# nlamprian/ICP

Hardware: AMD Instinct MI355X
Metric: ICP iterations/sec at |F|=|M|=16384, |R|=256 (higher is better)
Workload: dtype f32

## Files before the change

icp_amd/csrc/icp_search.h:

```cpp
#pragma once
#include "icp_kernels.h"

static __device__ __forceinline__ float sum4 (float4 v) { return ((v.x + v.y) + v.z) + v.w; }
static __device__ __forceinline__ uint32_t ks_hole_bit (float4 mg) { return (mg.x == 0.f && mg.y == 0.f && mg.z == 0.f) ? 0x80000000u : 0u; }

#define KS_SPLIT LPQ
#define KS_QPW (64 / KS_SPLIT)
#define KS_TILE 1024u
#ifndef ICP_S2_DEPTH16
#define ICP_S2_DEPTH16 8u
#endif
#ifndef ICP_S2_UNCOND
#define ICP_S2_UNCOND 128u
#endif
#ifndef ICP_S1_ORIGIN_LIST
#define ICP_S1_ORIGIN_LIST 1
#endif
#ifndef ICP_OL_STAGED_MIN
#define ICP_OL_STAGED_MIN 32u
#endif
#ifndef ICP_S1_SEED
#define ICP_S1_SEED 1
#endif
#ifndef ICP_S1_REJECT_MIN_NR
#define ICP_S1_REJECT_MIN_NR 1024u
#endif

typedef float float2v __attribute__ ((ext_vector_type (2)));

struct k_search_args {
    const float *gM, *gR; icp_reg_state *gst; const double *gmom;
    uint32_t m, nr, side, tpr_magic, nb, check_flags;
    icp_params p;
};
#define KS_PARAMS_OFFSET offsetof (k_search_args, p)
static_assert (KS_PARAMS_OFFSET == 4 * 8 + 6 * 4, "k_search: four pointers and six dwords in front of icp_params");
static_assert (KS_PARAMS_OFFSET % alignof (icp_params) == 0, "kernel-argument layout: icp_params follows the scalars without padding");
static __device__ __forceinline__ const icp_params *ks_params_from_kernarg ()
{
    unsigned long long a_ = (unsigned long long) __builtin_amdgcn_kernarg_segment_ptr () + KS_PARAMS_OFFSET;
    asm volatile ("" : "+s"(a_));
    return (const icp_params *) (const icp_params __attribute__ ((address_space (4))) *) a_;
}
#ifndef ICP_HOME_MODE
#define ICP_HOME_MODE 1
#endif

// ... 210 lines not shown
static __device__ __forceinline__ void fused_moment_task (uint32_t nb, uint32_t ps, uint32_t &k, uint32_t &g, bool &live)
{
    constexpr uint32_t nrow = NT / 16;
    const uint32_t row = threadIdx.x >> 4, ng = (nb + 127u) / 128u, ntask = ICP_NMOM * ng;
    const uint32_t task = min (ps * nrow + row, ntask - 1u);
    if (ng == 1) { k = task; g = 0u; } else if (ng == 2) { k = task >> 1; g = task & 1u; } else { k = task / ng; g = task - k * ng; }
    live = ps * nrow + row < ntask;
}
template <int NT>
static __device__ __forceinline__ void fused_moment_loads (const double *mom, uint32_t nb, uint32_t ps, double *a)
{
    uint32_t k, g; bool live;
    fused_moment_task<NT> (nb, ps, k, g, live);
    const double *src = mom + (size_t) k * nb;
    const uint32_t l = threadIdx.x & 15u;
#pragma unroll
    for (int q = 0; q < 8; ++q) a[q] = 0.0;
    if (live) {
        if (nb & 127u) {
#pragma unroll
            for (int q = 0; q < 8; ++q) {
                const uint32_t i = g * 128u + l + 16u * q;
                const double t = src[min (i, nb - 1u)];
                a[q] = (i < nb) ? t : 0.0;
            }
        } else {
#pragma unroll
            for (int q = 0; q < 8; ++q) a[q] = src[g * 128u + l + 16u * q];
        }
    }
}

struct ff_no_hook { __device__ void operator() (const float *) const {} };
template <int NG, int NT, int ROT, bool LEAN = false, bool REJ = false, typename AFTER = ff_no_hook>
static __device__ bool fused_finalize_block (const icp_params &p, const double *mom, uint32_t nb, uint32_t check, uint32_t sv,
                                             const double *a0, icp_fin_result *res, double (*s_l1)[NG], double *s_t,
                                             const double *gl1 = nullptr, icp_reg_state *direct = nullptr, AFTER after = AFTER (),
                                             uint32_t pending_unless_done = 1u, unsigned long long *mirror = nullptr, bool progress = false,
                                             icp_reg_state *final_dst = nullptr, icp_reg_state *host_dst = nullptr, icp_reg_state *prev_dst = nullptr)
{
    constexpr uint32_t nrow = NT / 16;
    const uint32_t tid = threadIdx.x, lane = tid & 63u, l = tid & 15u, row = tid >> 4;
    const uint32_t ng = (nb + 127u) / 128u;
    const uint32_t ntask = ICP_NMOM * ng, npass = (ntask + nrow - 1u) / nrow;
    auto pass = [&] (uint32_t ps, const double *a) {
        uint32_t k, g; bool live;
        fused_moment_task<NT> (nb, ps, k, g, live);
        FF_STAMP (13)
        double v = row_tree8_d (a);
        if (nb == 1) v = a[0];
        if (ng == 2) {
            const double o = __shfl_down (v, 16);
            if (l == 0 && !(row & 1u) && live) s_t[k] = (v + 0.0) + (o + 0.0);
        } else if (l == 0 && live) { if (ng == 1) s_t[k] = v; else s_l1[k][g] = v; }
    };
    if (gl1 == nullptr) {
        pass (0u, a0);
        for (uint32_t ps = 1; ps < npass; ++ps) {
            double a[8];
            fused_moment_loads<NT> (mom, nb, ps, a);
            pass (ps, a);
        }
    }
    if (check && __builtin_amdgcn_readlane ((int) sv, (int) ICP_ST_DW (done))) return false;
    FF_STAMP (9)
    if (ng > 2) {
        __syncthreads ();
        if (row < 20) {
            const uint32_t k = min (row, (uint32_t) ICP_NMOM - 1u);
            double a[8];
#pragma unroll
            for (int q = 0; q < 8; ++q) {
// ... 75 lines not shown
                        *reinterpret_cast<f4u *> (dst + 4) = f4u { Tprev[4], Tprev[5], Tprev[6], Tprev[7] };
                    }
                    if (mirror) {
                        if (done) {
                            if (final_dst) store_image (final_dst);
                            if (host_dst) { store_image (host_dst); __threadfence_system (); }
                            icp_mirror_store (mirror, ICP_MIRROR_WORD (p.epoch, kprev + 1u, 1u) | (host_dst ? ICP_MIRROR_FINAL : 0ull));
                            if (progress && p.run_flag) {
                                p.run_flag[blockIdx.y] = p.epoch;
                                if (p.track_seq) __hip_atomic_store (p.track_seq, p.seq_value, __ATOMIC_RELEASE, __HIP_MEMORY_SCOPE_AGENT);
                            }
                        } else if (progress) icp_mirror_store (mirror, ICP_MIRROR_WORD (p.epoch, kprev + 1u, 0u));
                    }
                }
            }
        } else if (lane == 0) {
            float Tn[8], Rn[9];
            if (none) icp_identity_step (Tprev, Rprev, S, means, Tk, Tn, Rn, Rk, iters);
            else icp_compose_pure (Tprev, Rprev, Tk, Rkin, ROT != 1, Tn, Rn, Rk);
#pragma unroll
            for (int k = 0; k < 8; ++k) { res->T[k] = Tn[k]; res->Tk[k] = Tk[k]; res->means[k] = means[k]; }
#pragma unroll
            for (int k = 0; k < 9; ++k) { res->R[k] = Rn[k]; res->Rk[k] = Rk[k]; }
#pragma unroll
            for (int k = 0; k < 11; ++k) res->S[k] = S[k];
            res->sum_w = sw; res->pm_iters = (uint32_t) iters; res->k = kprev + 1u; res->pad0 = 0.f; res->pending = 0u;
            res->reserved0 = 0u; res->reserved1 = 0u;
            res->done = (p.check && icp_check_converged (Tk, p.tan_half_thr, p.trans_thr)) ? 1u : 0u;
            if (prev_dst) {
#pragma unroll
                for (int k = 0; k < 8; ++k) prev_dst->T[k] = Tprev[k];
            }
        }
    }
    __syncthreads ();
    return true;
}

static __device__ __forceinline__ void fin_result_to_state (const icp_fin_result *res, icp_reg_state *st, uint32_t pending)
{
    static_assert (sizeof (icp_reg_state) / 4 <= 64, "the state is published by one wave");
    const uint32_t t = threadIdx.x;
    if (t < sizeof (icp_reg_state) / 4) {
        uint32_t v = reinterpret_cast<const uint32_t *> (res)[t];
        if (t == offsetof (icp_reg_state, pending) / 4) v = pending;
        reinterpret_cast<uint32_t *> (st)[t] = v;
    }
}

template <int LPQ>
static __device__ __forceinline__ void ks_list_tail (const char *XQb, uint32_t o, uint32_t je, uint32_t alast, uint32_t cb0, uint32_t ntrips, float qx, float qy, float qz,
                                                     float qr, float qg, float qb, float alpha, float dr, uint32_t b, uint32_t lane, uint32_t ss, float &best2, uint32_t &bj)
{
    const float2v vq_xr = { qx, qr }, vq_yg = { qy, qg }, vq_zb = { qz, qb };
    constexpr uint32_t CPT = 16u / KS_SPLIT, BD = KS_SPLIT == 16 ? 2u : 1u;
    const uint32_t nch = (je - o + 15u) >> 4, nchw = (ntrips + CPT - 1u) / CPT;
    const icp_params *pl = ks_params_from_kernarg ();
    typedef float4 __attribute__ ((address_space (1))) *gf4;
    const float4 *LBq = (const float4 *) (gf4) pl->LB + (size_t) b * 3u * pl->nlb + 3u * (o >> 4);
    const float inf_ = __builtin_inff ();
    float lim = (alpha > 0.f && dr >= 0.f && dr < inf_) ? __uint_as_float (__float_as_uint (dr) + 1u) : inf_;
    const bool bounds = alpha > 0.f;
    for (uint32_t cb = cb0; cb < nchw; cb += BD * KS_SPLIT) {
        lim = fminf (lim, ks_grp_min_f<KS_SPLIT> (best2));
        float4 bx[BD][3];
#pragma unroll
        for (uint32_t j = 0; j < BD; ++j) {
// ... 124 lines not shown
        const bool odd = (lane & 2u) != 0u;
        const unsigned long long keep = odd ? k4[2 * j + 1] : k4[2 * j], send = odd ? k4[2 * j] : k4[2 * j + 1];
        k2[j] = min64 (keep, xchg_dpp (send, std::integral_constant<int, 0x4E> {}));
    }
    {
        const bool odd = (lane & 4u) != 0u;
        const unsigned long long keep = odd ? k2[1] : k2[0], send = odd ? k2[0] : k2[1];
        k1 = min64 (keep, xchg_lane (send, lane ^ 4u));
    }
    k1 = min64 (k1, xchg_lane (k1, lane ^ 8u));
    k1 = min64 (k1, xchg_lane (k1, lane ^ 16u));
    k1 = min64 (k1, xchg_lane (k1, lane ^ 32u));
    k1 = xchg_lane (k1, (lane & 56u) | (lane >> 3));
    dmin = __uint_as_float ((uint32_t) (k1 >> 32)); jmin = (uint32_t) k1;
    {
        uint32_t nl = (je - o + 7u) >> 3;
        nl = max (nl, (uint32_t) __builtin_amdgcn_update_dpp (0, (int) nl, 0x140, 0xF, 0xF, true));
        nl = max (nl, (uint32_t) __builtin_amdgcn_update_dpp ((int) nl, (int) nl, 0x142, 0xA, 0xF, false));
        nl = max (nl, (uint32_t) __builtin_amdgcn_update_dpp ((int) nl, (int) nl, 0x143, 0xC, 0xF, false));
        const uint32_t ntrips = (uint32_t) __builtin_amdgcn_readlane ((int) nl, 63);
        if (__builtin_expect (ntrips > ICP_S2W_UNCOND / 8u, 0)) {
            const uint32_t ss = lane & 7u;
            float best2 = dmin; uint32_t bj = 0xFFFFFFFFu;
            const float4 a4 = s_qa[qe], c4 = s_qc[qe];
            ks_list_tail<8> (XQb, o, je, (max (je, 1u) - 1u) << 5, ICP_S2W_UNCOND / 16u, ntrips, a4.x, a4.y, a4.z, c4.x, c4.y, c4.z, alpha, dr, b, lane, ss, best2, bj);
            const uint32_t pos = bj != 0xFFFFFFFFu ? min (o + ss + bj * 8u, max (je, 1u) - 1u) : jmin;
            const float d2 = ks_grp_min_f<8> (best2);
            jmin = ks_grp_min_u<8> (best2 == d2 ? pos : 0xFFFFFFFFu);
            dmin = d2;
        }
    }
}

template <int LPQ>
static __device__ __forceinline__ void ks_stage2_lanes (const char *XQb, uint32_t o, uint32_t n, bool valid, float qx, float qy, float qz, float qr, float qg, float qb,
                                                        float alpha, float dr, uint32_t b, uint32_t lane, uint32_t ss, float &dmin, uint32_t &jmin)
{
    float best2 = __builtin_inff (); uint32_t bj = 0xFFFFFFFFu;
    const float2v vq_xr = { qx, qr }, vq_yg = { qy, qg }, vq_zb = { qz, qb };
    {
        constexpr uint32_t KS_DEPTH = (KS_SPLIT == 16) ? ICP_S2_DEPTH16 : 4u;
        const uint32_t je = valid ? o + n : o;
        uint32_t nl = (je - o + KS_SPLIT - 1u) / KS_SPLIT;
        if (KS_SPLIT == 8) nl = max (nl, (uint32_t) __builtin_amdgcn_update_dpp (0, (int) nl, 0x140, 0xF, 0xF, true));
        nl = max (nl, (uint32_t) __builtin_amdgcn_update_dpp ((int) nl, (int) nl, 0x142, 0xA, 0xF, false));
        nl = max (nl, (uint32_t) __builtin_amdgcn_update_dpp ((int) nl, (int) nl, 0x143, 0xC, 0xF, false));
        const uint32_t ntrips = (uint32_t) __builtin_amdgcn_readlane ((int) nl, 63);
        const uint32_t alast = (max (je, 1u) - 1u) << 5;
        constexpr uint32_t KS_UNC = ICP_S2_UNCOND / KS_SPLIT;
        const uint32_t ntr0 = (ICP_S2_UNCOND == 0u || ntrips <= 2u * KS_UNC) ? ntrips : KS_UNC;
        for (uint32_t tb = 0; tb < ntr0; tb += KS_DEPTH) {
            const uint32_t a0 = (o + ss + tb * KS_SPLIT) << 5, nt = min (KS_DEPTH, ntr0 - tb);
            float4 g[KS_DEPTH], c[KS_DEPTH];
#pragma unroll
            for (uint32_t t = 0; t < KS_DEPTH; ++t) {
                if (t >= nt) break;
                const char *rec = XQb + min (a0 + t * (KS_SPLIT * 32u), alast);
                g[t] = *reinterpret_cast<const float4 *> (rec); c[t] = *reinterpret_cast<const float4 *> (rec + 16);
            }
#pragma unroll
            for (uint32_t t = 0; t < KS_DEPTH; ++t) {
                if (t >= nt) break;
                KS_CAND (g[t], c[t], tb + t);
            }
        }
        if (__builtin_expect (ntrips > ntr0, 0))
            ks_list_tail<LPQ> (XQb, o, je, alast, ICP_S2_UNCOND / 16u, ntrips, qx, qy, qz, qr, qg, qb, alpha, dr, b, lane, ss, best2, bj);
        if (bj != 0xFFFFFFFFu) bj = min (o + ss + bj * KS_SPLIT, max (je, 1u) - 1u);
        if (je == o) { best2 = __builtin_inff (); bj = 0xFFFFFFFFu; }
    }
    dmin = ks_grp_min_f<KS_SPLIT> (best2);
    jmin = ks_grp_min_u<KS_SPLIT> (best2 == dmin ? bj : 0xFFFFFFFFu);
}

template <bool FUSED, bool CHAIN, int MINW, int LPQ, bool OWNER, bool PRUNE, bool REJ>
static __device__ __forceinline__ void ks_epilogue (const icp_params &p, float4 *s_qa, uint4 *s_qb, const float4 *s_qc, const uint32_t *s_slot, double (*s_mom)[64], float *s_w, const float4 *R4, const char *XQb,
                                                    uint32_t b, uint32_t m, uint32_t nr, uint32_t check_flags, uint32_t tid, uint32_t lane, uint32_t slice, uint32_t tile_id,
                                                    uint32_t qe, uint32_t ss, uint32_t i, bool valid, uint32_t o, uint32_t n, uint32_t rstar, float dr, float dmin, uint32_t jmin,
                                                    float qx, float qy, float qz)
{
    if (ss == 0u) {
        const bool empty = (n == 0u);
        s_qa[qe] = make_float4 (qx, qy, qz, empty ? dr : dmin);
        s_qb[qe] = make_uint4 (empty ? rstar : ((jmin == 0xFFFFFFFFu) ? o : jmin), rstar, (valid ? 1u : 0u) | (empty ? 2u : 0u), i);
    }
    __syncthreads ();
    if (slice == 0u) {
        const float4 qa = s_qa[lane]; const uint4 qb = s_qb[lane];
        const uint32_t eo = (PRUNE && ICP_S1_ORIGIN_LIST) ? s_slot[lane] : lane;
        const bool v = (qb.z & 1u) != 0u, empty = (qb.z & 2u) != 0u;
        const float ex = qa.x, ey = qa.y, ez = qa.z, d = p.dist_scale * qa.w;
        const uint32_t ei = qb.w;
        float w = 0.f, f0 = 0.f, f1 = 0.f, f2 = 0.f;
        bool acc = v;
        if (v) {
            uint32_t id;
            if (empty) {
                const float4 nn = R4[2 * (size_t) qb.x];
                const uint32_t *rsrc = p.rep_src;
                if constexpr (MINW == 4) {
                    typedef uint32_t __attribute__ ((address_space (1))) *gu32;
                    rsrc = (const uint32_t *) (gu32) ks_params_from_kernarg ()->rep_src;
                }
                id = rsrc[(size_t) b * nr + qb.x]; f0 = nn.x; f1 = nn.y; f2 = nn.z;
            } else {
                const char *rec = XQb + (qb.x << 5);
                const float4 wg = *reinterpret_cast<const float4 *> (rec), wc = *reinterpret_cast<const float4 *> (rec + 16);
                f0 = wg.x; f1 = wg.z; f2 = wc.x; id = __float_as_uint (wc.z);
            }
            w = p.weighted ? 100.f / (100.f + d) : 1.f;
            if constexpr (REJ) {
                bool rej = false;
                if (p.reject & 1u)
                    rej = (__float_as_uint (s_qc[lane].w) >> 31) != 0u || (f0 == 0.f && f1 == 0.f && f2 == 0.f);
                if (p.reject & ICP_REJECT_DIST_ON) {
                    const float gx = ex - f0, gy = ey - f1, gz = ez - f2;
                    rej = rej || !(((gx * gx + gy * gy) + gz * gz) <= p.reject_d2);
                }
                if (rej) { w = 0.f; acc = false; }
            }
            icp_dist_id di; di.dist = d; di.id = id;
            const icp_params *pe = &p;
            if constexpr (MINW == 2 && !OWNER) {
                            pe = ks_params_from_kernarg ();
            }
            typedef char __attribute__ ((address_space (1))) *gchar;
            char *o_nn = (char *) (gchar) reinterpret_cast<char *> (pe->nn_id + (size_t) b * m), *o_pf = (char *) (gchar) reinterpret_cast<char *> (pe->PF + (size_t) b * m);
            char *o_pm = (char *) (gchar) reinterpret_cast<char *> (pe->PM + (size_t) b * m), *o_rid = (char *) (gchar) reinterpret_cast<char *> (pe->rid + (size_t) b * m);
            const bool emit = !FUSED || (check_flags & 8u);
            if (emit) {
                *reinterpret_cast<icp_dist_id *> (o_nn + (ei << 3)) = di;
                *reinterpret_cast<float4 *> (o_pf + (ei << 4)) = make_float4 (f0, f1, f2, w);
                *reinterpret_cast<float4 *> (o_pm + (ei << 4)) = make_float4 (ex, ey, ez, d);
            }
            if (emit || PRUNE) *reinterpret_cast<uint32_t *> (o_rid + (ei << 2)) = qb.y;
        }
        if constexpr (FUSED) {
            double W = (double) w;
            double g0 = acc ? (double) f0 : 0.0, g1 = acc ? (double) f1 : 0.0, g2 = acc ? (double) f2 : 0.0;
            double q0 = (double) ex, q1 = (double) ey, q2 = (double) ez;
            if (!acc) { W = 0.0; q0 = q1 = q2 = 0.0; }
// ... 82 lines not shown
                                                     uint32_t gt_lg1, uint32_t ss, uint32_t t0_, uint32_t npair_, uint32_t cmask_, float &best, uint32_t &bid)
{
    const uint32_t ngt_ = (npair_ + KS_SPLIT - 1u) / KS_SPLIT;
    const float2v vqx = { qx, qx }, vqy = { qy, qy }, vqz = { qz, qz }, vqr = { qr, qr }, vqg = { qg, qg }, vqb = { qb, qb };
    const float2v va = { alpha, alpha };
    for (uint32_t t = 0; t * KS_SPLIT < ngt_; ++t) {
        unsigned long long bal = __ballot ((cmask_ >> t) & 1u);
        if (bal == 0ull) continue;
        bal |= bal >> 32; bal |= bal >> 16;
        if (KS_SPLIT == 8) bal |= bal >> 8;
        uint32_t need = (uint32_t) bal & ((1u << KS_SPLIT) - 1u);
        while (need) {
            const uint32_t sg = (uint32_t) __builtin_ctz (need);
            need &= need - 1u;
            const uint32_t gl = sg + KS_SPLIT * t;
            const uint32_t P = (KS_SPLIT == 8 && gt_lg1) ? (((4u * (gl >> (gt_lg1 - 1u)) + (ss >> 1)) << gt_lg1) + 2u * (gl & ((1u << (gt_lg1 - 1u)) - 1u)) + (ss & 1u))
                                                          : gl * KS_SPLIT + ss;
            if (P < npair_) {
                const uint32_t P3 = pair0 + __umul24 (P, 3u);
                float4 A = s_pair[P3], B = s_pair[P3 + 1], C = s_pair[P3 + 2];
                float2v x = { A.x, A.y }, y = { A.z, A.w }, z = { B.x, B.y }, r = { B.z, B.w }, g = { C.x, C.y }, bb = { C.z, C.w };
                float2v dx = vqx - x, dy = vqy - y, dz = vqz - z, dr = vqr - r, dg = vqg - g, db = vqb - bb;
                float2v geo = __builtin_elementwise_fma (dz, dz, __builtin_elementwise_fma (dy, dy, dx * dx));
                float2v pho = __builtin_elementwise_fma (db, db, __builtin_elementwise_fma (dg, dg, dr * dr));
                float2v d = __builtin_elementwise_fma (va, pho, geo);
                const uint32_t r0 = t0_ + 2u * P;
                if (d.x < best) { best = d.x; bid = r0; }
                if (d.y < best) { best = d.y; bid = r0 + 1u; }
            }
        }
    }
}

template <bool FUSED, bool CHAIN, int MINW, int LPQ, bool OWNER = false, int ROT = 1, int TILE = 1024, bool SINGLE = false, bool S2W = false, bool HOSTRUN = false,
          bool REJ = false>
__global__ __launch_bounds__ (64 * LPQ, TILE == 256 ? 8 : MINW) void k_search (const float *gM, const float *gR, icp_reg_state *gst, const double *gmom,
                                                              uint32_t m, uint32_t nr, uint32_t side, uint32_t tpr_magic,
                                                              uint32_t nb, uint32_t check_flags, icp_params p)
{
    constexpr uint32_t KT = (uint32_t) TILE;
    constexpr bool MASKED = (TILE == 256) && !SINGLE && (MINW == 4);
    if constexpr (SINGLE) __builtin_assume (nr <= KT);
    if constexpr (MASKED) __builtin_assume (nr > KT && nr <= 32u * KT);
    const uint32_t b = blockIdx.y, check = check_flags & 1u;
    icp_reg_state *st = (CHAIN && !(check_flags & 2u)) ? gst + (size_t) b * 2 : gst + b;
#ifdef ICP_DBG_STAMPS
    { const uint32_t tid = threadIdx.x; unsigned long long t_; asm volatile ("s_memtime %0\n\ts_waitcnt lgkmcnt(0)" : "=s"(t_) :: "memory");
      KS_STAMP_STORE (8) }
#endif

    constexpr uint32_t NBUF = MASKED ? 2u : 1u, PB = 3u * KT / 2u, BB = 2u * (KT / 16u);
    __shared__ float4 s_pair[NBUF * PB];
    __shared__ uint2 s_on[(MASKED && OWNER) ? 1 : KT];
    __shared__ uint32_t s_tmask;
    __shared__ uint32_t s_ovote;
    __shared__ float4 s_box[NBUF * BB];
    __shared__ float4 s_tbox[(MINW == 4 && !SINGLE) ? 2 * 32 : 2];
    __shared__ float s_w[64];
    __shared__ float4 s_qc[64];
    __shared__ float4 s_qa[64];
    __shared__ uint4 s_qb[64];
    __shared__ uint32_t s_slot[(ICP_S1_SEED && ICP_S1_ORIGIN_LIST && MINW == 4) ? 64 : 1];
    __shared__ double s_mom[FUSED ? ICP_NMOM : 1][64];
    __shared__ icp_fin_result s_fin;
    __shared__ double s_l1[CHAIN ? ICP_NMOM : 1][CHAIN ? 32 : 1];
    __shared__ double s_t[ICP_NMOM];

    const uint32_t tid = threadIdx.x, lane = tid & 63u;
    const uint32_t slice = __builtin_amdgcn_readfirstlane (tid >> 6);
    const uint32_t qe = slice * KS_QPW + lane / KS_SPLIT, ss = lane & (KS_SPLIT - 1u);
    const bool qwave = CHAIN ? slice == 0u : slice == KS_SPLIT - 1u;
    constexpr bool OWNER_LISTS = OWNER && MINW == 2;
    const uint32_t tile_id = OWNER_LISTS ? blockIdx.x : (FUSED && (MINW == 2 || (check_flags & 64u))) ? ks_tile_of_block (blockIdx.x, nb) : blockIdx.x;
    const uint32_t iq = OWNER_LISTS ? blockIdx.x * 64u + lane :
                        FUSED ? fused_query_index (m, side, tpr_magic, tile_id, lane)
                              : (blockIdx.x >> 1) * 128u + 2u * lane + (blockIdx.x & 1u);

    const float4 *M4 = reinterpret_cast<const float4 *> (gM + (size_t) b * m * 8);
    const float4 *R4 = reinterpret_cast<const float4 *> (gR + (size_t) b * nr * 8);

    uint32_t sv = OWNER ? 0u : state_load_lanes (st);
    uint32_t run_over = 0u;
    if constexpr (CHAIN) {
        static_assert (ICP_ST_DW (T) == 0 && ICP_ST_DW (Tk) == 8 && ICP_ST_DW (R) == 16 && ICP_ST_DW (Rk) == 25 && ICP_ST_DW (reserved0) == 60, "state layout");
        if (check_flags & 16u) {
            constexpr unsigned long long ones = (1ull << 3) | (1ull << 7) | (1ull << 11) | (1ull << 15) | (1ull << 16) | (1ull << 20) | (1ull << 24) |
                                                (1ull << 25) | (1ull << 29) | (1ull << 33);
            if (lane < ICP_ST_DW (reserved0)) sv = ((ones >> lane) & 1ull) ? 0x3F800000u : 0u;
        }
    }
    double ma0[8];
    if constexpr (CHAIN) fused_moment_loads<64 * LPQ> (gmom + (size_t) b * 2 * ICP_NMOM * nb, nb, 0u, ma0);
    float *s_pairf = reinterpret_cast<float *> (s_pair);
    const uint32_t tn0 = min (KT, nr);
    float4 rg[2], rc[2]; uint2 ron[2];
    uint32_t ht = 0u, tnH = 0u;
#pragma unroll
    for (int u = 0; u < 2; ++u) {
        uint32_t k = tid + (uint32_t) u * 64u * KS_SPLIT;
// ... 42 lines not shown
    }
    const float4 *GBt = p.GB + (size_t) b * 2 * (p.n16 + p.n1k) + (KS_SPLIT == 8 ? 0u : 2u * p.n16);
    const uint32_t nbox0 = 2u * ((tn0 + 2u * KS_SPLIT - 1u) / (2u * KS_SPLIT));
    float4 boxv = make_float4 (0.f, 0.f, 0.f, 0.f);
    if (!MASKED && prune && tid < nbox0) boxv = GBt[tid];
    const uint32_t nboxH = 2u * ((tnH + 2u * KS_SPLIT - 1u) / (2u * KS_SPLIT));
    if (MASKED && ICP_HOME_MODE != 3 && prune && tid < nboxH) boxv = GBt[2u * (ht * KT / (2u * KS_SPLIT)) + tid];
    float T[8];
#pragma unroll
    for (int k = 0; k < 8; ++k) T[k] = state_lane_f (sv, ICP_ST_DW (T) + k);
    if constexpr (PRUNE && !OWNER) {
        if (seed_cell != 0xFFFFFFFFu && __builtin_amdgcn_readlane ((int) sv, (int) ICP_ST_DW (k)) == 0) seed = seed_cell | (ICP_S1_ORIGIN_LIST ? 0x40000000u : 0u);
    }
    icp_reg_state *sout = CHAIN ? p.cst + (size_t) b * 2 + (p.slot ^ 1u) : st;
    if constexpr (!OWNER && !CHAIN) {
        const uint32_t done_ = (uint32_t) __builtin_amdgcn_readlane ((int) sv, (int) ICP_ST_DW (done));
        if (p.hmirror && blockIdx.x == 0 && tid == 0 && !(FUSED && done_))
            icp_mirror_store (p.hmirror + b, ICP_MIRROR_WORD (p.epoch, (uint32_t) __builtin_amdgcn_readlane ((int) sv, (int) ICP_ST_DW (k)), done_));
    }
    if constexpr (CHAIN && HOSTRUN) { if (run_over) return; }
    if (!OWNER && check && __builtin_amdgcn_readlane ((int) sv, (int) ICP_ST_DW (done))) {
        if constexpr (CHAIN) {
            if (blockIdx.x == 0 && tid < sizeof (icp_reg_state) / 4) reinterpret_cast<uint32_t *> (sout)[tid] = sv;
        }
        return;
    }
    if constexpr (!S2W) asm volatile ("" : "+v"(mgv), "+v"(mcv));
    float4 mg = make_float4 (mgv.x, mgv.y, mgv.z, mgv.w), mc = make_float4 (mcv.x, mcv.y, mcv.z, mcv.w);
    if (iq >= m) { mg = make_float4 (0.f, 0.f, 0.f, 1.f); mc = mg; }
    uint32_t hbit = 0u;
    if constexpr (REJ && !OWNER) { hbit = ks_hole_bit (mg); if constexpr (CHAIN) asm volatile ("" : "+v"(hbit)); }
    const float4 *XQ4 = reinterpret_cast<const float4 *> (p.XQ + (size_t) b * m * 8);
    const char *XQb = reinterpret_cast<const char *> (XQ4);
#pragma unroll
    for (int u = 0; u < 2; ++u) {
        uint32_t k = tid + (uint32_t) u * 64u * KS_SPLIT;
        if (!MASKED && k < tn0) {
            float *dst = s_pairf + (k >> 1) * 12u + (k & 1u);
            dst[0] = rg[u].x; dst[2] = rg[u].y; dst[4] = rg[u].z; dst[6] = rc[u].x; dst[8] = rc[u].y; dst[10] = rc[u].z;
            if constexpr (!OWNER && !MASKED) s_on[k] = ron[u];
        }
    }
    if (!MASKED && prune && tid < nbox0) s_box[tid] = boxv;
    auto home_to_lds = [&] () {
        if (tid < tnH) {
            float *dst = s_pairf + PB * 4u + (tid >> 1) * 12u + (tid & 1u);
            dst[0] = rg[0].x; dst[2] = rg[0].y; dst[4] = rg[0].z; dst[6] = rc[0].x; dst[8] = rc[0].y; dst[10] = rc[0].z;
        }
        if (prune && tid < nboxH) s_box[BB + tid] = boxv;
    };
    if constexpr (MASKED) {
        if (ICP_HOME_MODE == 1) home_to_lds ();
        if constexpr (!OWNER) { if (tid < tnH) s_on[tid] = ron[0]; }
    }
    if (MASKED && tid == 0) s_tmask = 0u;
    if (PRUNE && ICP_S1_ORIGIN_LIST && tid == 0) s_ovote = 0u;
    if constexpr (MINW == 4 && !SINGLE) {
        if (prune && nr > KT && tid < 2u * p.n1k) s_tbox[tid] = p.GB[(size_t) b * 2 * (p.n16 + p.n1k) + 2u * p.n16 + tid];
    }
    bool handed = false;
    if constexpr (CHAIN) {
        const bool pending = __builtin_amdgcn_readlane ((int) sv, (int) ICP_ST_DW (pending)) != 0;
        if (pending) {
            auto hand_over = [&] (const float *Tn) {
                float tx, ty, tz;
                icp_transform_point (Tn, mg.x, mg.y, mg.z, tx, ty, tz);
                s_qa[lane] = make_float4 (tx, ty, tz, __uint_as_float (iq));
                s_qc[lane] = make_float4 (mc.x, mc.y, mc.z, __uint_as_float (seed | hbit));
            };
            fused_finalize_block<32, 64 * LPQ, ROT, true, REJ> (p, gmom + (size_t) b * 2 * ICP_NMOM * nb, nb, 0u, sv, ma0, &s_fin, s_l1, s_t, nullptr,
                                                           blockIdx.x == 0 ? sout : nullptr, hand_over, 1u,
                                                           (HOSTRUN && blockIdx.x == 0 && p.hmirror) ? p.hmirror + b : nullptr, HOSTRUN, HOSTRUN ? p.st + b : nullptr,
                                                           (HOSTRUN && p.hstate) ? p.hstate + b : nullptr, (HOSTRUN && p.st_prev) ? p.st_prev + b : nullptr);
            handed = true;
            KS_STAMP (9)
            if (s_fin.done) return;
        } else if (blockIdx.x == 0 && tid < sizeof (icp_reg_state) / 4) {
            reinterpret_cast<uint32_t *> (sout)[tid] = (tid == offsetof (icp_reg_state, pending) / 4) ? 1u : sv;
        }
    }
    if (qwave && !handed) {
        float tx = mg.x, ty = mg.y, tz = mg.z;
        if constexpr (!OWNER) icp_transform_point (T, mg.x, mg.y, mg.z, tx, ty, tz);
        if constexpr (PRUNE && ICP_S1_ORIGIN_LIST) {
            const bool hole = mg.x == 0.f && mg.y == 0.f && mg.z == 0.f;
            const float4 ha = make_float4 (tx, ty, tz, __uint_as_float (iq)), hc = make_float4 (mc.x, mc.y, mc.z, __uint_as_float (hole ? (seed | 0x80000000u) : seed));
            s_qa[lane] = ha; s_qc[lane] = hc; s_slot[lane] = lane;
            const unsigned long long hb = __ballot (hole);
            if (__builtin_expect (hb != 0ull, 0)) {
                const unsigned long long lt = (1ull << lane) - 1ull;
                const uint32_t pos = hole ? 64u - (uint32_t) __builtin_popcountll (hb) + (uint32_t) __builtin_popcountll (hb & lt) : (uint32_t) __builtin_popcountll (~hb & lt);
                s_qa[pos] = ha; s_qc[pos] = hc; s_slot[pos] = lane;
            }
        } else {
            s_qa[lane] = make_float4 (tx, ty, tz, __uint_as_float (iq));
            s_qc[lane] = make_float4 (mc.x, mc.y, mc.z, __uint_as_float (seed | hbit));
        }
    }
    float qx = 0.f, qy = 0.f, qz = 0.f, qr = 0.f, qg = 0.f, qb = 0.f;
    uint32_t i = 0u; bool valid = false;
    const float alpha = p.a;
    KS_STAMP (0)

    float best = __builtin_inff (), s1_lim = __builtin_inff (); uint32_t bid = 0xFFFFFFFFu;
    uint32_t n_origin = 0u;
    if constexpr (MASKED) {
// ... 162 lines not shown
                float4 A = s_pair[3 * P], B = s_pair[3 * P + 1], C = s_pair[3 * P + 2];
                float2v x = { A.x, A.y }, y = { A.z, A.w }, z = { B.x, B.y }, r = { B.z, B.w }, g = { C.x, C.y }, bb = { C.z, C.w };
                float2v dx = vqx - x, dy = vqy - y, dz = vqz - z, dr = vqr - r, dg = vqg - g, db = vqb - bb;
                float2v geo = __builtin_elementwise_fma (dz, dz, __builtin_elementwise_fma (dy, dy, dx * dx));
                float2v pho = __builtin_elementwise_fma (db, db, __builtin_elementwise_fma (dg, dg, dr * dr));
                float2v d = __builtin_elementwise_fma (va, pho, geo);
                const uint32_t r0 = t0 + 2u * P;
                if (d.x < best) { best = d.x; bid = r0; }
                if (d.y < best) { best = d.y; bid = r0 + 1u; }
            }
        }
    }
    KS_STAMP (14)
    if constexpr (PRUNE && ICP_S1_ORIGIN_LIST) {
        if (prune && __builtin_expect (n_origin != 0u, 0))
            ks_origin_section<KS_SPLIT, PB> (s_pair, &s_ovote, n_origin, nr, b, slice, tid, qx, qy, qz, qr, qg, qb, alpha, s1_lim, lane, ss, best, bid);
    }
    KS_KEEP (best, bid)
    KS_STAMP (2)
    const float dr = ks_grp_min_f<KS_SPLIT> (best);
    const bool named = PRUNE ? (best == dr && dr < __builtin_inff ()) : (best == dr);
    uint32_t rstar = ks_grp_min_u<KS_SPLIT> (named ? bid : 0xFFFFFFFFu);
    if (rstar == 0xFFFFFFFFu) rstar = 0u;
    if constexpr (OWNER_LISTS) {
        ks_owner_lists_tail (p, s_qb, b, m, nb, lane, slice, qe, ss, valid, rstar);
        return;
    } else if constexpr (OWNER) {
        if (ss == 0u && valid) p.owner[(size_t) b * m + i] = rstar;
        return;
    }
    KS_KEEP (dr, rstar)
    KS_STAMP (3)
    uint32_t o, n;
    if constexpr (MINW == 2) { const uint2 on = s_on[rstar]; o = on.x; n = on.y; }
    else if constexpr (MASKED) {
        if (rstar / KT == ht) { const uint2 on = s_on[rstar - ht * KT]; o = on.x; n = on.y; asm volatile ("" : "+v"(o), "+v"(n)); }
        else { o = gO[rstar]; n = gN[rstar]; }
    }
    else if (nr <= KT) { const uint2 on = s_on[rstar]; o = on.x; n = on.y; asm volatile ("" : "+v"(o), "+v"(n)); }
    else { o = gO[rstar]; n = gN[rstar]; }

    float dmin; uint32_t jmin;
    if constexpr (S2W) {
        static_assert (MINW == 4 && LPQ == 8 && !OWNER, "lanes = candidates: the dense search variants");
        ks_stage2_wave (XQb, o, n, valid, rstar, qx, qy, qz, qr, qg, qb, alpha, dr, b, lane, s_qa, s_qc, qe, dmin, jmin);
    } else ks_stage2_lanes<LPQ> (XQb, o, n, valid, qx, qy, qz, qr, qg, qb, alpha, dr, b, lane, ss, dmin, jmin);
    KS_KEEP (dmin, jmin)
    KS_STAMP (5)
    ks_epilogue<FUSED, CHAIN, MINW, LPQ, OWNER, PRUNE, REJ> (p, s_qa, s_qb, s_qc, s_slot, s_mom, s_w, R4, XQb, b, m, nr, check_flags, tid, lane, slice, tile_id, qe, ss, i, valid, o, n, rstar, dr, dmin, jmin,
                                                        qx, qy, qz);
}


static inline uint32_t icp_tpr_magic (uint32_t side)
{
    const uint32_t tpr = side >> 3;
    return tpr ? (uint32_t) ((1ull << 32) / tpr + 1ull) : 0u;
}
#define KS_FLAGS(p) ((uint32_t) ((p).check ? 1u : 0u) | ((p).emit ? 8u : 0u) | ((p).warm_seed ? 32u : 0u) | ((p).xcdmap ? 64u : 0u))
#define KS_ARGS p.M, p.R, p.st, (const double *) p.mom, p.m, p.nr, p.side, icp_tpr_magic (p.side), p.nb, KS_FLAGS (p), p
#define KS_CHAIN_ARGS p.M, p.R, p.cst + p.slot, (const double *) p.mom + (size_t) p.slot * ICP_NMOM * p.nb, p.m, p.nr, p.side, icp_tpr_magic (p.side), p.nb, KS_FLAGS (p), p

template <bool REJ>
void ks_launch_dense (const icp_params &p, hipStream_t s)
{
    const bool t256 = icp_dense_tile (p) == 256u, multi = p.nr > 256u;
    if (p.fused) {
        if (p.s2wave && multi && t256) hipLaunchKernelGGL ((k_search<true, false, 4, 8, false, 1, 256, false, true, false, REJ>), dim3 (p.nb, p.batch), dim3 (512), 0, s, KS_ARGS);
        else if (p.s2wave && t256) hipLaunchKernelGGL ((k_search<true, false, 4, 8, false, 1, 256, true, true, false, REJ>), dim3 (p.nb, p.batch), dim3 (512), 0, s, KS_ARGS);
        else if (p.s2wave) hipLaunchKernelGGL ((k_search<true, false, 4, 8, false, 1, 1024, false, true, false, REJ>), dim3 (p.nb, p.batch), dim3 (512), 0, s, KS_ARGS);
        else if (multi && t256) hipLaunchKernelGGL ((k_search<true, false, 4, 8, false, 1, 256, false, false, false, REJ>), dim3 (p.nb, p.batch), dim3 (512), 0, s, KS_ARGS);
        else if (t256) hipLaunchKernelGGL ((k_search<true, false, 4, 8, false, 1, 256, true, false, false, REJ>), dim3 (p.nb, p.batch), dim3 (512), 0, s, KS_ARGS);
        else hipLaunchKernelGGL ((k_search<true, false, 4, 8, false, 1, 1024, false, false, false, REJ>), dim3 (p.nb, p.batch), dim3 (512), 0, s, KS_ARGS);
    } else {
        if (p.s2wave && multi && t256) hipLaunchKernelGGL ((k_search<false, false, 4, 8, false, 1, 256, false, true, false, REJ>), dim3 (2 * p.nwg, p.batch), dim3 (512), 0, s, KS_ARGS);
        else if (p.s2wave && t256) hipLaunchKernelGGL ((k_search<false, false, 4, 8, false, 1, 256, true, true, false, REJ>), dim3 (2 * p.nwg, p.batch), dim3 (512), 0, s, KS_ARGS);
        else if (p.s2wave) hipLaunchKernelGGL ((k_search<false, false, 4, 8, false, 1, 1024, false, true, false, REJ>), dim3 (2 * p.nwg, p.batch), dim3 (512), 0, s, KS_ARGS);
        else if (multi && t256) hipLaunchKernelGGL ((k_search<false, false, 4, 8, false, 1, 256, false, false, false, REJ>), dim3 (2 * p.nwg, p.batch), dim3 (512), 0, s, KS_ARGS);
        else if (t256) hipLaunchKernelGGL ((k_search<false, false, 4, 8, false, 1, 256, true, false, false, REJ>), dim3 (2 * p.nwg, p.batch), dim3 (512), 0, s, KS_ARGS);
        else hipLaunchKernelGGL ((k_search<false, false, 4, 8, false, 1, 1024, false, false, false, REJ>), dim3 (2 * p.nwg, p.batch), dim3 (512), 0, s, KS_ARGS);
    }
}

// ... 26 lines not shown
```

Measured before the change: 113,800.

## Stage the 3x3 neighbourhood's model lists in LDS during the finalize idle wait

While the lead wave runs the lean fused finalize, the other waves now prefetch the XQ records of the up to nine representative cells around the tile's home cell into a shared-memory buffer, provided each list is short enough. Stage 2 reads candidates from this LDS copy when every lane of a wave has a staged list, and the epilogue reads the winning record from LDS rather than global memory. This hides global latency inside an existing idle window but costs extra LDS per block (about 31 KB), which may lower occupancy, and it repacks the slot index into the high bits of the list count.

Result: slower. 109,100 (-4.1%).

```diff
diff --git a/icp_amd/csrc/icp_search.h b/icp_amd/csrc/icp_search.h
--- a/icp_amd/csrc/icp_search.h
+++ b/icp_amd/csrc/icp_search.h
@@ -13,6 +13,12 @@
 #ifndef ICP_S2_UNCOND
 #define ICP_S2_UNCOND 128u
 #endif
+#define ICP_HOME_CAP 110u
+#define ICP_HOME_SLOTS 9u
+#ifndef ICP_HOME_LISTS
+#define ICP_HOME_LISTS 1
+#endif
+static_assert (ICP_HOME_CAP <= ICP_S2_UNCOND && ICP_HOME_SLOTS * 2u * ICP_HOME_CAP < (1u << 26), "home lists: scanned unconditionally; a place in them fits the hand-off word");
 #ifndef ICP_S1_ORIGIN_LIST
 #define ICP_S1_ORIGIN_LIST 1
 #endif
@@ -289,12 +295,14 @@
 }
 
 struct ff_no_hook { __device__ void operator() (const float *) const {} };
-template <int NG, int NT, int ROT, bool LEAN = false, bool REJ = false, typename AFTER = ff_no_hook>
+struct ff_no_idle { __device__ void operator() () const {} };
+template <int NG, int NT, int ROT, bool LEAN = false, bool REJ = false, typename AFTER = ff_no_hook, typename IDLE = ff_no_idle>
 static __device__ bool fused_finalize_block (const icp_params &p, const double *mom, uint32_t nb, uint32_t check, uint32_t sv,
                                              const double *a0, icp_fin_result *res, double (*s_l1)[NG], double *s_t,
                                              const double *gl1 = nullptr, icp_reg_state *direct = nullptr, AFTER after = AFTER (),
                                              uint32_t pending_unless_done = 1u, unsigned long long *mirror = nullptr, bool progress = false,
-                                             icp_reg_state *final_dst = nullptr, icp_reg_state *host_dst = nullptr, icp_reg_state *prev_dst = nullptr)
+                                             icp_reg_state *final_dst = nullptr, icp_reg_state *host_dst = nullptr, icp_reg_state *prev_dst = nullptr,
+                                             IDLE idle = IDLE ())
 {
     constexpr uint32_t nrow = NT / 16;
     const uint32_t tid = threadIdx.x, lane = tid & 63u, l = tid & 15u, row = tid >> 4;
@@ -436,7 +444,7 @@
                 for (int k = 0; k < 8; ++k) prev_dst->T[k] = Tprev[k];
             }
         }
-    }
+    } else if constexpr (LEAN) idle ();
     __syncthreads ();
     return true;
 }
@@ -627,9 +635,10 @@
     }
 }
 
-template <int LPQ>
+template <int LPQ, bool HOME = false>
 static __device__ __forceinline__ void ks_stage2_lanes (const char *XQb, uint32_t o, uint32_t n, bool valid, float qx, float qy, float qz, float qr, float qg, float qb,
-                                                        float alpha, float dr, uint32_t b, uint32_t lane, uint32_t ss, float &dmin, uint32_t &jmin)
+                                                        float alpha, float dr, uint32_t b, uint32_t lane, uint32_t ss, float &dmin, uint32_t &jmin,
+                                                        const float4 *s_home = nullptr, uint32_t hs = 0u)
 {
     float best2 = __builtin_inff (); uint32_t bj = 0xFFFFFFFFu;
     const float2v vq_xr = { qx, qr }, vq_yg = { qy, qg }, vq_zb = { qz, qb };
@@ -644,7 +653,27 @@
         const uint32_t alast = (max (je, 1u) - 1u) << 5;
         constexpr uint32_t KS_UNC = ICP_S2_UNCOND / KS_SPLIT;
         const uint32_t ntr0 = (ICP_S2_UNCOND == 0u || ntrips <= 2u * KS_UNC) ? ntrips : KS_UNC;
-        for (uint32_t tb = 0; tb < ntr0; tb += KS_DEPTH) {
+        [[maybe_unused]] bool from_lds = false;
+        if constexpr (HOME) {
+            static_assert (KS_DEPTH * KS_SPLIT >= ICP_HOME_CAP, "a staged list is one batch");
+            from_lds = __ballot (hs == 0u && je != o) == 0ull;
+            if (from_lds) {
+                const uint32_t hb = (hs ? hs - 1u : 0u) * (2u * ICP_HOME_CAP), last = max (je - o, 1u) - 1u, nt = min (KS_DEPTH, ntrips);
+                float4 g[KS_DEPTH], c[KS_DEPTH];
+#pragma unroll
+                for (uint32_t t = 0; t < KS_DEPTH; ++t) {
+                    if (t >= nt) break;
+                    const uint32_t pos = hb + min (ss + t * KS_SPLIT, last);
+                    g[t] = s_home[pos]; c[t] = s_home[pos + ICP_HOME_CAP];
+                }
+#pragma unroll
+                for (uint32_t t = 0; t < KS_DEPTH; ++t) {
+                    if (t >= nt) break;
+                    KS_CAND (g[t], c[t], t);
+                }
+            }
+        }
+        for (uint32_t tb = from_lds ? ntr0 : 0u; tb < ntr0; tb += KS_DEPTH) {
             const uint32_t a0 = (o + ss + tb * KS_SPLIT) << 5, nt = min (KS_DEPTH, ntr0 - tb);
             float4 g[KS_DEPTH], c[KS_DEPTH];
 #pragma unroll
@@ -668,15 +697,20 @@
     jmin = ks_grp_min_u<KS_SPLIT> (best2 == dmin ? bj : 0xFFFFFFFFu);
 }
 
-template <bool FUSED, bool CHAIN, int MINW, int LPQ, bool OWNER, bool PRUNE, bool REJ>
+template <bool FUSED, bool CHAIN, int MINW, int LPQ, bool OWNER, bool PRUNE, bool REJ, bool HOME = false>
 static __device__ __forceinline__ void ks_epilogue (const icp_params &p, float4 *s_qa, uint4 *s_qb, const float4 *s_qc, const uint32_t *s_slot, double (*s_mom)[64], float *s_w, const float4 *R4, const char *XQb,
                                                     uint32_t b, uint32_t m, uint32_t nr, uint32_t check_flags, uint32_t tid, uint32_t lane, uint32_t slice, uint32_t tile_id,
                                                     uint32_t qe, uint32_t ss, uint32_t i, bool valid, uint32_t o, uint32_t n, uint32_t rstar, float dr, float dmin, uint32_t jmin,
-                                                    float qx, float qy, float qz)
+                                                    float qx, float qy, float qz, const float4 *s_home = nullptr, uint32_t hs = 0u)
 {
     if (ss == 0u) {
         const bool empty = (n == 0u);
         s_qa[qe] = make_float4 (qx, qy, qz, empty ? dr : dmin);
+        if constexpr (HOME) {
+            const uint32_t wpos = (jmin == 0xFFFFFFFFu) ? o : jmin;
+            const uint32_t hl = (hs && !empty) ? ((hs - 1u) * (2u * ICP_HOME_CAP) + (wpos - o) + 1u) << 2 : 0u;
+            s_qb[qe] = make_uint4 (empty ? rstar : wpos, rstar, (valid ? 1u : 0u) | (empty ? 2u : 0u) | hl, i);
+        } else
         s_qb[qe] = make_uint4 (empty ? rstar : ((jmin == 0xFFFFFFFFu) ? o : jmin), rstar, (valid ? 1u : 0u) | (empty ? 2u : 0u), i);
     }
     __syncthreads ();
@@ -699,9 +733,14 @@
                 }
                 id = rsrc[(size_t) b * nr + qb.x]; f0 = nn.x; f1 = nn.y; f2 = nn.z;
             } else {
+                if (HOME && (qb.z >> 2)) {
+                    const float4 wg = s_home[(qb.z >> 2) - 1u], wc = s_home[(qb.z >> 2) - 1u + ICP_HOME_CAP];
+                    f0 = wg.x; f1 = wg.z; f2 = wc.x; id = __float_as_uint (wc.z);
+                } else {
                 const char *rec = XQb + (qb.x << 5);
                 const float4 wg = *reinterpret_cast<const float4 *> (rec), wc = *reinterpret_cast<const float4 *> (rec + 16);
                 f0 = wg.x; f1 = wg.z; f2 = wc.x; id = __float_as_uint (wc.z);
+                }
             }
             w = p.weighted ? 100.f / (100.f + d) : 1.f;
             if constexpr (REJ) {
@@ -850,6 +889,22 @@
     }
 }
 
+struct ks_home_cell { uint32_t cx, cy, lgx, nrx, nry; bool on; };
+static __device__ __forceinline__ ks_home_cell ks_home_cell_of (uint32_t m, uint32_t side, uint32_t tpr_magic, uint32_t tile_id)
+{
+    const icp_params *po = ks_params_from_kernarg ();
+    const uint32_t i0 = (uint32_t) __builtin_amdgcn_readfirstlane ((int) min (fused_query_index (m, side, tpr_magic, tile_id, 0u), m - 1u));
+    const uint32_t nrx = po->nrx, side_magic = po->side_magic, cw = po->cellw_magic, ch = po->cellh_magic;
+    ks_home_cell h = { 0u, 0u, 0u, nrx, po->nry, false };
+    if (side_magic && nrx && (nrx & (nrx - 1u)) == 0u) {
+        const uint32_t y = __umulhi (i0, side_magic), x = i0 - y * side;
+        h.cy = ch ? __umulhi (y, ch) : y; h.cx = cw ? __umulhi (x, cw) : x;
+        h.lgx = 31u - (uint32_t) __builtin_clz (nrx);
+        h.on = true;
+    }
+    return h;
+}
+
 template <bool FUSED, bool CHAIN, int MINW, int LPQ, bool OWNER = false, int ROT = 1, int TILE = 1024, bool SINGLE = false, bool S2W = false, bool HOSTRUN = false,
           bool REJ = false>
 __global__ __launch_bounds__ (64 * LPQ, TILE == 256 ? 8 : MINW) void k_search (const float *gM, const float *gR, icp_reg_state *gst, const double *gmom,
@@ -883,6 +938,8 @@
     __shared__ icp_fin_result s_fin;
     __shared__ double s_l1[CHAIN ? ICP_NMOM : 1][CHAIN ? 32 : 1];
     __shared__ double s_t[ICP_NMOM];
+    constexpr bool HOME = ICP_HOME_LISTS && CHAIN && MINW == 2 && LPQ == 16 && !OWNER && !HOSTRUN;
+    __shared__ float4 s_home[HOME ? ICP_HOME_SLOTS * 2u * ICP_HOME_CAP : 1u];
 
     const uint32_t tid = threadIdx.x, lane = tid & 63u;
     const uint32_t slice = __builtin_amdgcn_readfirstlane (tid >> 6);
@@ -991,12 +1048,19 @@
     if constexpr (REJ && !OWNER) { hbit = ks_hole_bit (mg); if constexpr (CHAIN) asm volatile ("" : "+v"(hbit)); }
     const float4 *XQ4 = reinterpret_cast<const float4 *> (p.XQ + (size_t) b * m * 8);
     const char *XQb = reinterpret_cast<const char *> (XQ4);
+    ks_home_cell hc = {};
+    if constexpr (HOME) hc = ks_home_cell_of (m, side, tpr_magic, tile_id);
 #pragma unroll
     for (int u = 0; u < 2; ++u) {
         uint32_t k = tid + (uint32_t) u * 64u * KS_SPLIT;
         if (!MASKED && k < tn0) {
             float *dst = s_pairf + (k >> 1) * 12u + (k & 1u);
             dst[0] = rg[u].x; dst[2] = rg[u].y; dst[4] = rg[u].z; dst[6] = rc[u].x; dst[8] = rc[u].y; dst[10] = rc[u].z;
+            if constexpr (HOME) {
+                const uint32_t dx = (k & (hc.nrx - 1u)) - hc.cx + 1u, dy = (k >> hc.lgx) - hc.cy + 1u;
+                const bool pend_ = __builtin_amdgcn_readlane ((int) sv, (int) ICP_ST_DW (pending)) != 0;
+                if (hc.on && pend_ && dx <= 2u && dy <= 2u && ron[u].y - 1u < ICP_HOME_CAP) ron[u].y |= (dy * 3u + dx + 1u) << 28;
+            }
             if constexpr (!OWNER && !MASKED) s_on[k] = ron[u];
         }
     }
@@ -1027,10 +1091,36 @@
                 s_qa[lane] = make_float4 (tx, ty, tz, __uint_as_float (iq));
                 s_qc[lane] = make_float4 (mc.x, mc.y, mc.z, __uint_as_float (seed | hbit));
             };
+            auto stage_home = [&] () {
+                if constexpr (HOME) {
+                    const ks_home_cell hw = ks_home_cell_of (m, side, tpr_magic, tile_id);
+                    if (!hw.on) return;
+                    constexpr uint32_t NTH = 64u * (LPQ - 1u), NROUND = (ICP_HOME_SLOTS * 2u * ICP_HOME_CAP + NTH - 1u) / NTH;
+                    static_assert (NROUND == 3u, "three rounds, written out (an indexed private array would be put in LDS)");
+                    auto fetch = [&] (uint32_t r, float4 &v) -> uint32_t {
+                        const uint32_t u = tid - 64u + r * NTH;
+                        const uint32_t sl = u / (2u * ICP_HOME_CAP);
+                        if (sl >= ICP_HOME_SLOTS) return 0xFFFFFFFFu;
+                        const uint32_t sy = (sl * 11u) >> 5, kx = hw.cx + (sl - 3u * sy) - 1u, ky = hw.cy + sy - 1u;
+                        if (kx >= hw.nrx || ky >= hw.nry) return 0xFFFFFFFFu;
+                        const uint2 on = s_on[min ((ky << hw.lgx) + kx, nr - 1u)];
+                        const uint32_t rec = (u % (2u * ICP_HOME_CAP)) >> 1, half = u & 1u;
+                        if ((on.y >> 28) != sl + 1u || rec >= (on.y & 0x0FFFFFFFu)) return 0xFFFFFFFFu;
+                        v = XQ4[2u * (size_t) (on.x + rec) + half];
+                        return sl * (2u * ICP_HOME_CAP) + half * ICP_HOME_CAP + rec;
+                    };
+                    float4 v0, v1, v2;
+                    const uint32_t d0 = fetch (0u, v0), d1 = fetch (1u, v1), d2 = fetch (2u, v2);
+                    if (d0 != 0xFFFFFFFFu) s_home[d0] = v0;
+                    if (d1 != 0xFFFFFFFFu) s_home[d1] = v1;
+                    if (d2 != 0xFFFFFFFFu) s_home[d2] = v2;
+                }
+            };
             fused_finalize_block<32, 64 * LPQ, ROT, true, REJ> (p, gmom + (size_t) b * 2 * ICP_NMOM * nb, nb, 0u, sv, ma0, &s_fin, s_l1, s_t, nullptr,
                                                            blockIdx.x == 0 ? sout : nullptr, hand_over, 1u,
                                                            (HOSTRUN && blockIdx.x == 0 && p.hmirror) ? p.hmirror + b : nullptr, HOSTRUN, HOSTRUN ? p.st + b : nullptr,
-                                                           (HOSTRUN && p.hstate) ? p.hstate + b : nullptr, (HOSTRUN && p.st_prev) ? p.st_prev + b : nullptr);
+                                                           (HOSTRUN && p.hstate) ? p.hstate + b : nullptr, (HOSTRUN && p.st_prev) ? p.st_prev + b : nullptr,
+                                                           stage_home);
             handed = true;
             KS_STAMP (9)
             if (s_fin.done) return;
@@ -1259,7 +1349,9 @@
     KS_KEEP (dr, rstar)
     KS_STAMP (3)
     uint32_t o, n;
-    if constexpr (MINW == 2) { const uint2 on = s_on[rstar]; o = on.x; n = on.y; }
+    uint32_t hs = 0u;
+    if constexpr (HOME) { const uint2 on = s_on[rstar]; o = on.x; n = on.y & 0x0FFFFFFFu; hs = on.y >> 28; }
+    else if constexpr (MINW == 2) { const uint2 on = s_on[rstar]; o = on.x; n = on.y; }
     else if constexpr (MASKED) {
         if (rstar / KT == ht) { const uint2 on = s_on[rstar - ht * KT]; o = on.x; n = on.y; asm volatile ("" : "+v"(o), "+v"(n)); }
         else { o = gO[rstar]; n = gN[rstar]; }
@@ -1271,11 +1363,11 @@
     if constexpr (S2W) {
         static_assert (MINW == 4 && LPQ == 8 && !OWNER, "lanes = candidates: the dense search variants");
         ks_stage2_wave (XQb, o, n, valid, rstar, qx, qy, qz, qr, qg, qb, alpha, dr, b, lane, s_qa, s_qc, qe, dmin, jmin);
-    } else ks_stage2_lanes<LPQ> (XQb, o, n, valid, qx, qy, qz, qr, qg, qb, alpha, dr, b, lane, ss, dmin, jmin);
+    } else ks_stage2_lanes<LPQ, HOME> (XQb, o, n, valid, qx, qy, qz, qr, qg, qb, alpha, dr, b, lane, ss, dmin, jmin, s_home, hs);
     KS_KEEP (dmin, jmin)
     KS_STAMP (5)
-    ks_epilogue<FUSED, CHAIN, MINW, LPQ, OWNER, PRUNE, REJ> (p, s_qa, s_qb, s_qc, s_slot, s_mom, s_w, R4, XQb, b, m, nr, check_flags, tid, lane, slice, tile_id, qe, ss, i, valid, o, n, rstar, dr, dmin, jmin,
-                                                        qx, qy, qz);
+    ks_epilogue<FUSED, CHAIN, MINW, LPQ, OWNER, PRUNE, REJ, HOME> (p, s_qa, s_qb, s_qc, s_slot, s_mom, s_w, R4, XQb, b, m, nr, check_flags, tid, lane, slice, tile_id, qe, ss, i, valid, o, n, rstar, dr, dmin, jmin,
+                                                        qx, qy, qz, s_home, hs);
 }
 
 
```
